# ZhangLearning/llm-message-queue

Measured on AMD Instinct MI355X. Metric: requests/sec + p99 enqueue->dispatch latency, 4-tier mix at 1/2/4/8 backends, higher is better.
Workload: dtype bf16

## Files before the change

### csrc/kernels/gemm_kernels.h

```cpp
#pragma once

#include <hip/hip_runtime.h>
#include <stdint.h>

#include <type_traits>

#include "fp8_decode.h"
#include "sample_noise.h"

namespace llmq {

typedef __attribute__((ext_vector_type(8))) short gm_bf16x8;
typedef __attribute__((ext_vector_type(4))) float gm_f32x4;
typedef __attribute__((ext_vector_type(4))) unsigned int gm_u32x4;

constexpr int GM_BM = 256, GM_BN = 256, GM_BK = 64, GM_THREADS = 512;
constexpr int GM_HALF_BYTES = 128 * GM_BK * 2;
constexpr int GM_BUF_BYTES = 4 * GM_HALF_BYTES;
constexpr int GM_LDS_BYTES = 2 * GM_BUF_BYTES;
constexpr int GM_GROUP_M = 8;

enum { GM_EPI_STORE = 0, GM_EPI_SWIGLU = 2, GM_EPI_ROPE = 3, GM_EPI_ARGMAX = 4, GM_EPI_RESID = 5,
       GM_EPI_RESID_LDS = 6, GM_EPI_RESID_PRE = 7, GM_EPI_RESID_RMS = 8, GM_EPI_SAMPLE = 9 };
constexpr int GM_LDS_SPARE = 32768;
template <int EPI>
constexpr int gm_lds_bytes() { return EPI == GM_EPI_RESID_PRE ? GM_LDS_BYTES + GM_LDS_SPARE : GM_LDS_BYTES; }

enum {
  GM_DIAG_NONE = 0,
  GM_DIAG_SKIP_A2 = 1,
  GM_DIAG_NO_LDS_READ = 2,
  GM_DIAG_NO_DMA = 3,
  GM_DIAG_CLOCK = 4,
  GM_DIAG_CLOCK_NO_DMA = 5,
  GM_DIAG_L2_PANELS = 6
};

struct GmSide {
  float* pv;
  int32_t* pi;
  union {
    float* rpart;
    const float* inv_temp;
  };
  union {
    int* rticket;
    const uint32_t* key;
  };
  float* rscale;
  float reps;
};

struct GmRope {
  const int32_t* pos;
  const int32_t* slot;
  const float* cos_t;
  const float* sin_t;
  uint16_t* q;
  uint16_t* kc;
  uint16_t* vc;
  int Hq, Hkv, max_ctx, n_slots;
};
enum { GM_A0 = 0, GM_A1 = 1, GM_B0 = 2, GM_B1 = 3 };

__device__ __forceinline__ uint16_t gm_f2bf(float f) {
  uint32_t u = __float_as_uint(f);
  u += 0x7fffu + ((u >> 16) & 1u);
  return (uint16_t)(u >> 16);
}

__device__ __forceinline__ void gm_load_row_scales(const float* __restrict__ rs, int row0, int fq,
                                                   gm_f32x4 (&sc)[2][4]) {
  if (rs) {
#pragma unroll
    for (int mh = 0; mh < 2; ++mh)
#pragma unroll
      for (int m = 0; m < 4; ++m)
        sc[mh][m] = *reinterpret_cast<const gm_f32x4*>(rs + row0 + mh * 64 + m * 16 + fq * 4);
  } else {
#pragma unroll
    for (int mh = 0; mh < 2; ++mh)
#pragma unroll
      for (int m = 0; m < 4; ++m) sc[mh][m] = gm_f32x4{1.f, 1.f, 1.f, 1.f};
  }
}

#define GM_CPOL_SC1 16

struct GmSplit {
  int full;
  float* ws;
  int* cnt;
};

typedef __attribute__((address_space(3))) void* gm_lds_ptr;
typedef gm_f32x4 gm_acc_t[2][4][2][2];

__device__ __forceinline__ void gm_stage(__amdgpu_buffer_rsrc_t rs, uint32_t v0, uint32_t v1, uint32_t soff,
                                         uint8_t* smem, uint32_t dst0, uint32_t dst1) {
  __builtin_amdgcn_raw_ptr_buffer_load_lds(rs, (gm_lds_ptr)(smem + dst0), 16, v0, soff, 0, 0);
  __builtin_amdgcn_raw_ptr_buffer_load_lds(rs, (gm_lds_ptr)(smem + dst1), 16, v1, soff, 0, 0);
}

#define GM_LGKM(N) asm volatile("s_waitcnt lgkmcnt(" #N ")" ::: "memory")
#define GM_VMCNT(N) asm volatile("s_waitcnt vmcnt(%0)" ::"n"(N) : "memory")
#define GM_FENCE() __builtin_amdgcn_sched_barrier(0)
#define GM_BARRIER()                  \
  do {                                \
    GM_FENCE();                       \
    __builtin_amdgcn_s_barrier();     \
    GM_FENCE();                       \
  } while (0)

typedef __attribute__((ext_vector_type(2))) unsigned int gf_u32x2;
template <int OFF>
__device__ __forceinline__ gf_u32x2 gf_lds_read_b64(uint32_t addr) {
  gf_u32x2 r;
  asm volatile("ds_read_b64 %0, %1 offset:%2" : "=v"(r) : "v"(addr), "n"(OFF) : "memory");
  return r;
}

template <int PER>
__device__ __forceinline__ int gm_xcd_run_start(int b, int count) {
  const int n = PER * count;
  const int xcd = b & 7, q8 = n >> 3, r8 = n & 7;
  return xcd < r8 ? xcd * (q8 + 1) : r8 * (q8 + 1) + (xcd - r8) * q8;
}

struct GmTile {
  int tm, tn;
  int pid;
// ... 54 lines not shown
    for (int spin = 0; spin < (1 << 24); ++spin) {
      if (__hip_atomic_load(cnt + 1, __ATOMIC_RELAXED, __HIP_MEMORY_SCOPE_AGENT)) break;
      __builtin_amdgcn_s_sleep(2);
    }
    GM_VMCNT(0);
    __hip_atomic_store(cnt, 0, __ATOMIC_RELAXED, __HIP_MEMORY_SCOPE_AGENT);
    __hip_atomic_store(cnt + 1, 0, __ATOMIC_RELAXED, __HIP_MEMORY_SCOPE_AGENT);
  }
  __syncthreads();
#pragma unroll
  for (int a = 0; a < 2; ++a)
#pragma unroll
    for (int b = 0; b < 4; ++b)
#pragma unroll
      for (int c = 0; c < 2; ++c)
#pragma unroll
        for (int d = 0; d < 2; ++d)
        {
          const int i = ((a * 4 + b) * 4 + c * 2 + d) * GM_THREADS + tid;
          acc[a][b][c][d] += __builtin_bit_cast(gm_f32x4, __builtin_amdgcn_raw_buffer_load_b128(
                                 srs, i * 16, 0, GM_CPOL_SC1));
        }
  return false;
}


template <int EPI, int DIAG, bool FP8 = false>
__device__ __forceinline__ void gemm_tile(
    uint8_t* __restrict__ smem, const uint16_t* __restrict__ A, const void* __restrict__ W,
    const float* __restrict__ cs, uint16_t* __restrict__ C, int M, int N, int K, int group_m,
    const float* __restrict__ rs, const GmRope& rp, const GmSplit& sp, const GmSide& am, const int bid) {
  static_assert(!FP8 || (DIAG == GM_DIAG_NONE &&
                         (EPI == GM_EPI_STORE || EPI == GM_EPI_SWIGLU || EPI == GM_EPI_RESID_LDS)),
                "the FP8 form: STORE, SWIGLU and RESID_LDS, no diagnostics");
  constexpr int kBHalf = 128 * GM_BK * (FP8 ? 1 : 2);
  constexpr int kBuf = 2 * GM_HALF_BYTES + 2 * kBHalf;
  static_assert(2 * kBuf <= GM_LDS_BYTES, "operand buffers inside the launch's LDS");
  constexpr bool kStamp = DIAG == GM_DIAG_CLOCK || DIAG == GM_DIAG_CLOCK_NO_DMA;
  const int tiles_m = (M + GM_BM - 1) / GM_BM;
  const int tiles_n = N / GM_BN;
  const int nwg = tiles_m * tiles_n;
  const int full = sp.ws ? sp.full : nwg;
  const GmTile tile = gm_tile_coords(bid, tiles_m, tiles_n, nwg, full, group_m);
  const int pid = tile.pid, khalf = tile.khalf, tm = tile.tm, tn = tile.tn;

  const int tid = threadIdx.x;
  const int lane = tid & 63;
  const int w = __builtin_amdgcn_readfirstlane(tid >> 6);
  uint64_t st_t0 = 0, st_r0 = 0;
  if constexpr (kStamp) {
    st_t0 = __builtin_amdgcn_s_memtime();
    st_r0 = __builtin_amdgcn_s_memrealtime();
  }
  const int wr = w >> 2, wc = w & 3;

  const int srow = w * 8 + (lane >> 3);
  const int schunk = (lane & 7) ^ ((srow >> 1) & 7);
  const int brow = w * 16 + (lane >> 2);
  const int bchunk = (lane & 3) ^ ((brow >> 2) & 3);
  const __amdgpu_buffer_rsrc_t rsa = __builtin_amdgcn_make_buffer_rsrc((void*)A, 0, M * K * 2, 0x00020000);
  const __amdgpu_buffer_rsrc_t rsw =
      __builtin_amdgcn_make_buffer_rsrc((void*)W, 0, N * K * (FP8 ? 1 : 2), 0x00020000);
  uint32_t va[2][2], vb[2][FP8 ? 1 : 2];
  const int ltm = DIAG == GM_DIAG_L2_PANELS ? 0 : tm, ltn = DIAG == GM_DIAG_L2_PANELS ? 0 : tn;
#pragma unroll
  for (int h = 0; h < 2; ++h) {
#pragma unroll
    for (int i = 0; i < 2; ++i) {
      int row = ltm * GM_BM + i * 128 + h * 64 + srow;
      row = row < M ? row : M - 1;
      va[h][i] = (uint32_t)row * (uint32_t)K * 2u + (uint32_t)schunk * 16u;
      if constexpr (!FP8) {
        const int col = ltn * GM_BN + (2 * i + (w >> 2)) * 64 + h * 32 + (w & 3) * 8 + (lane >> 3);
        vb[h][i] = (uint32_t)col * (uint32_t)K * 2u + (uint32_t)schunk * 16u;
      }
    }
    if constexpr (FP8) {
      const int col = ltn * GM_BN + (brow >> 5) * 64 + h * 32 + (brow & 31);
      vb[h][0] = (uint32_t)col * (uint32_t)K + (uint32_t)bchunk * 16u;
    }
  }
  const uint32_t dst_i0 = (uint32_t)(w * 8) * 128u;
  const uint32_t dst_i1 = (uint32_t)(64 + w * 8) * 128u;
  const uint32_t dst_b = (uint32_t)(w * 16) * 64u;

  const uint32_t sbase = (uint32_t)(uintptr_t)(__attribute__((address_space(3))) uint8_t*)smem;
  const int fr = lane & 15, fq = lane >> 4;
  uint32_t aoff[2][2], boff[2][2];
#pragma unroll
  for (int kk = 0; kk < 2; ++kk) {
    const int c = fq + 4 * kk;
    aoff[0][kk] = (uint32_t)(wr * 64 + fr) * 128u + (uint32_t)((c ^ ((fr >> 1) & 7)) * 16);
    if constexpr (FP8)
      boff[0][kk] = (uint32_t)(2 * GM_HALF_BYTES) + (uint32_t)(wc * 32 + fr) * 64u +
                    (uint32_t)(((c >> 1) ^ ((fr >> 2) & 3)) * 16 + (c & 1) * 8);
    else
      boff[0][kk] = (uint32_t)(wc * 32 + fr) * 128u + (uint32_t)((c ^ ((fr >> 1) & 7)) * 16) + 2 * GM_HALF_BYTES;
    aoff[1][kk] = aoff[0][kk] + kBuf;
    boff[1][kk] = boff[0][kk] + kBuf;
  }

  gm_acc_t acc;
#pragma unroll
  for (int a = 0; a < 2; ++a)
#pragma unroll
    for (int b = 0; b < 4; ++b)
// ... 38 lines not shown
      _Pragma("unroll") for (int kk = 0; kk < 2; ++kk) {                                       \
        DST[0][kk] = gf_lds_read_b64<(NH) * kBHalf>(sbase + boff[BUF][kk]);                    \
        DST[1][kk] = gf_lds_read_b64<(NH) * kBHalf + 1024>(sbase + boff[BUF][kk]);             \
      }                                                                                        \
    } else {                                                                                   \
      _Pragma("unroll") for (int n = 0; n < 2; ++n)                                            \
        _Pragma("unroll") for (int kk = 0; kk < 2; ++kk)                                       \
          DST[n][kk] = *reinterpret_cast<const gm_bf16x8*>(smem + boff[BUF][kk] + (NH) * kBHalf + n * 2048); \
    }                                                                                          \
  } while (0)
#define GM_READ_B(BUF, NH) GM_READ_B_INTO(BUF, NH, bfr[NH])
#define GM_READ_B0_INTO(BUF, DST) GM_READ_B_INTO(BUF, 0, DST)

#define GM_MFMA_WITH(MH, NH, BREG)                                                             \
  do {                                                                                         \
    _Pragma("unroll") for (int kk = 0; kk < 2; ++kk) {                                         \
      gm_bf16x8 _b[2];                                                                         \
      _Pragma("unroll") for (int n = 0; n < 2; ++n) {                                          \
        if constexpr (FP8) _b[n] = sk_fp8x8_bf16(BREG[n][kk].x, BREG[n][kk].y);                \
        else _b[n] = BREG[n][kk];                                                              \
      }                                                                                        \
      _Pragma("unroll") for (int m = 0; m < 4; ++m)                                            \
        _Pragma("unroll") for (int n = 0; n < 2; ++n)                                          \
          acc[MH][m][NH][n] = __builtin_amdgcn_mfma_f32_16x16x32_bf16(af[m][kk], _b[n],        \
                                                                      acc[MH][m][NH][n], 0, 0, 0); \
    }                                                                                          \
  } while (0)

#define GM_PHASE_END(MH, NH, BREG)   \
  do {                               \
    GM_BARRIER();                    \
    GM_LGKM(0);                      \
    if constexpr (FP8) GM_FENCE();   \
    GM_MFMA_WITH(MH, NH, BREG);      \
    GM_BARRIER();                    \
  } while (0)

  constexpr int kDmaA = 2, kDmaB = FP8 ? 1 : 2;
  constexpr int kFlyA = 2 * kDmaA + kDmaB, kFlyB = kDmaA + 2 * kDmaB;

  if (wr == 1) __builtin_amdgcn_s_setprio(1);
  if constexpr (EPI == GM_EPI_RESID_PRE) {
    const int col0p = tn * GM_BN + wc * 64, row0p = tm * GM_BM + wr * 128;
    const __amdgpu_buffer_rsrc_t rsp =
        __builtin_amdgcn_make_buffer_rsrc((void*)C, 0, (uint32_t)M * (uint32_t)N * 2u, 0x00020000);
#pragma unroll
    for (int i = 0; i < 4; ++i) {
      const int r = i * 8 + (lane >> 3), c = lane & 7;
      const uint32_t vo = ((uint32_t)(row0p + r) * (uint32_t)N + (uint32_t)(col0p + c * 8)) * 2u;
      __builtin_amdgcn_raw_ptr_buffer_load_lds(rsp, (gm_lds_ptr)(smem + GM_LDS_BYTES + w * 4096 + i * 1024), 16,
                                               vo, 0, 0, 0);
    }
  }
  GM_STAGE(0, GM_B0, 0);
  GM_STAGE(0, GM_A0, 0);
  GM_STAGE(0, GM_B1, 0);
  GM_STAGE(0, GM_A1, 0);
  GM_STAGE(1, GM_B0, 1);
  GM_STAGE(1, GM_A0, 1);
  GM_STAGE(1, GM_B1, 1);
  GM_VMCNT(kFlyB);
  GM_BARRIER();
  GM_READ_B0_INTO(0, bfr[0]);
  if constexpr (DIAG >= GM_DIAG_SKIP_A2 && DIAG <= GM_DIAG_NO_DMA) {
    GM_READ_A(0, 0);
    GM_READ_B(0, 1);
    GM_READ_B0_INTO(1, b0y);
  }
  if (wr == 1) GM_BARRIER();

  int t = 0;
  constexpr bool kRdA = DIAG != GM_DIAG_NO_LDS_READ;
  constexpr bool kRdA2 = DIAG != GM_DIAG_SKIP_A2 && DIAG != GM_DIAG_NO_LDS_READ;
  constexpr bool kRdB = DIAG != GM_DIAG_NO_LDS_READ;
  constexpr bool kDma = DIAG != GM_DIAG_NO_DMA && DIAG != GM_DIAG_CLOCK_NO_DMA;
#define GM_D_READ_A(ON, B, H) do { if constexpr (ON) GM_READ_A(B, H); } while (0)
#define GM_D_READ_B(B, H) do { if constexpr (kRdB) GM_READ_B(B, H); } while (0)
#define GM_D_READ_B0(B, D) do { if constexpr (kRdB) GM_READ_B0_INTO(B, D); } while (0)
#define GM_D_STAGE(B, H, K) do { if constexpr (kDma) GM_STAGE(B, H, K); } while (0)
  for (; t < nt - 2; t += 2) {
    {
      GM_D_READ_A(kRdA, 0, 0); GM_D_STAGE(1, GM_A1, t + 1); GM_VMCNT(kFlyA); GM_PHASE_END(0, 0, bfr[0]);
      GM_D_READ_B(0, 1); GM_D_STAGE(0, GM_B0, t + 2); GM_VMCNT(kFlyB); GM_PHASE_END(0, 1, bfr[1]);
      GM_D_READ_A(kRdA2, 0, 1); GM_D_STAGE(0, GM_A0, t + 2); GM_VMCNT(kFlyA); GM_PHASE_END(1, 1, bfr[1]);
      GM_D_READ_B0(1, b0y); GM_D_STAGE(0, GM_B1, t + 2); GM_VMCNT(kFlyB); GM_PHASE_END(1, 0, bfr[0]);
      GM_D_READ_A(kRdA, 1, 0); GM_D_STAGE(0, GM_A1, t + 2); GM_VMCNT(kFlyA); GM_PHASE_END(0, 0, b0y);
      GM_D_READ_B(1, 1); GM_D_STAGE(1, GM_B0, t + 3); GM_VMCNT(kFlyB); GM_PHASE_END(0, 1, bfr[1]);
      GM_D_READ_A(kRdA2, 1, 1); GM_D_STAGE(1, GM_A0, t + 3); GM_VMCNT(kFlyA); GM_PHASE_END(1, 1, bfr[1]);
      GM_D_READ_B0(0, bfr[0]); GM_D_STAGE(1, GM_B1, t + 3); GM_VMCNT(kFlyB); GM_PHASE_END(1, 0, b0y);
    }
  }
  {
      GM_READ_A(0, 0); GM_STAGE(1, GM_A1, t + 1); GM_VMCNT(kFlyA); GM_PHASE_END(0, 0, bfr[0]);
      GM_READ_B(0, 1); GM_VMCNT(kDmaA + kDmaB); GM_PHASE_END(0, 1, bfr[1]);
      GM_READ_A(0, 1); GM_VMCNT(kDmaA); GM_PHASE_END(1, 1, bfr[1]);
      GM_READ_B0_INTO(1, b0y); GM_VMCNT(0); GM_PHASE_END(1, 0, bfr[0]);
      GM_READ_A(1, 0); GM_PHASE_END(0, 0, b0y);
      GM_READ_B(1, 1); GM_PHASE_END(0, 1, bfr[1]);
      GM_READ_A(1, 1); GM_PHASE_END(1, 1, bfr[1]);
      GM_PHASE_END(1, 0, b0y);
  }
  __builtin_amdgcn_s_setprio(0);
  if (wr == 0) GM_BARRIER();
#undef GM_D_READ_A
#undef GM_D_READ_B
#undef GM_D_READ_B0
#undef GM_D_STAGE
#undef GM_PHASE_END
#undef GM_MFMA_WITH
#undef GM_READ_B0_INTO
#undef GM_READ_B
#undef GM_READ_B_INTO
#undef GM_READ_A
#undef GM_STAGE

  if (khalf >= 0 && gm_split_join(smem, acc, sp, pid - full)) return;

  if constexpr (FP8) {
    const float* csp = cs + tn * GM_BN + wc * 64 + fr;
#pragma unroll
    for (int nh = 0; nh < 2; ++nh)
#pragma unroll
      for (int n = 0; n < 2; ++n) {
        const float s = csp[nh * 32 + n * 16];
#pragma unroll
        for (int mh = 0; mh < 2; ++mh)
#pragma unroll
          for (int m = 0; m < 4; ++m) acc[mh][m][nh][n] *= s;
      }
  }

  const int row0 = tm * GM_BM + wr * 128;
  if constexpr (EPI == GM_EPI_ARGMAX || EPI == GM_EPI_SAMPLE) {
    if constexpr (EPI == GM_EPI_SAMPLE) {
      const uint32_t col = (uint32_t)(tn * GM_BN + wc * 64 + fr);
#pragma unroll
      for (int mh = 0; mh < 2; ++mh)
#pragma unroll
        for (int m = 0; m < 4; ++m) {
          const int r4 = row0 + mh * 64 + m * 16 + fq * 4;
          const gm_f32x4 it = *reinterpret_cast<const gm_f32x4*>(am.inv_temp + r4);
          const gm_u32x4 ka = *reinterpret_cast<const gm_u32x4*>(am.key + 2 * r4);
          const gm_u32x4 kb = *reinterpret_cast<const gm_u32x4*>(am.key + 2 * r4 + 4);
#pragma unroll
          for (int j = 0; j < 4; ++j) {
            const uint32_t k0 = j < 2 ? ka[2 * j] : kb[2 * j - 4];
            const uint32_t k1 = j < 2 ? ka[2 * j + 1] : kb[2 * j - 3];
            if (it[j] != 0.f) {
#pragma unroll
              for (int nh = 0; nh < 2; ++nh)
#pragma unroll
                for (int n = 0; n < 2; ++n)
                  acc[mh][m][nh][n][j] = acc[mh][m][nh][n][j] * it[j] + sn_gumbel(k0, k1, col + nh * 32 + n * 16);
            }
          }
        }
// ... 31 lines not shown
    if (tid < GM_BM) {
      const int grow = tm * GM_BM + tid;
      float v = lv[tid * 4];
      int c = lc[tid * 4];
#pragma unroll
      for (int k = 1; k < 4; ++k)
        if (lv[tid * 4 + k] > v) { v = lv[tid * 4 + k]; c = lc[tid * 4 + k]; }
      if (grow < M) {
        am.pv[(int64_t)grow * tiles_n + tn] = v;
        am.pi[(int64_t)grow * tiles_n + tn] = tn * GM_BN + c;
      }
    }
  } else if constexpr (EPI == GM_EPI_RESID) {
    float* o = reinterpret_cast<float*>(smem + w * (32 * 68 * 4));
    const int col0 = tn * GM_BN + wc * 64;
    uint2 cres[2][2][8];
#pragma unroll
    for (int mh = 0; mh < 2; ++mh)
#pragma unroll
      for (int mp = 0; mp < 2; ++mp)
#pragma unroll
        for (int it = 0; it < 8; ++it) {
          const int qd = it * 64 + lane;
          const int grow = row0 + mh * 64 + mp * 32 + (qd >> 4);
          cres[mh][mp][it] = grow < M ? *reinterpret_cast<const uint2*>(C + (int64_t)grow * N + col0 + (qd & 15) * 4)
                                      : make_uint2(0u, 0u);
        }
#pragma unroll
    for (int mh = 0; mh < 2; ++mh)
#pragma unroll
      for (int mp = 0; mp < 2; ++mp) {
#pragma unroll
        for (int mm = 0; mm < 2; ++mm)
#pragma unroll
          for (int nh = 0; nh < 2; ++nh)
#pragma unroll
            for (int n = 0; n < 2; ++n)
#pragma unroll
              for (int j = 0; j < 4; ++j)
                o[(mm * 16 + fq * 4 + j) * 68 + nh * 32 + n * 16 + fr] = acc[mh][mp * 2 + mm][nh][n][j];
        GM_LGKM(0);
        __builtin_amdgcn_wave_barrier();
#pragma unroll
        for (int it = 0; it < 8; ++it) {
          const int qd = it * 64 + lane;
          const int r = qd >> 4, c4 = qd & 15;
          const int grow = row0 + mh * 64 + mp * 32 + r;
          const gm_f32x4 v = *reinterpret_cast<const gm_f32x4*>(o + r * 68 + c4 * 4);
          if (grow < M) {
            uint2* cp = reinterpret_cast<uint2*>(C + (int64_t)grow * N + col0 + c4 * 4);
            const uint2 cr = cres[mh][mp][it];
            const float r0 = __uint_as_float(cr.x << 16) + v[0], r1 = __uint_as_float(cr.x & 0xffff0000u) + v[1];
            const float r2 = __uint_as_float(cr.y << 16) + v[2], r3 = __uint_as_float(cr.y & 0xffff0000u) + v[3];
            *cp = make_uint2((uint32_t)gm_f2bf(r0) | ((uint32_t)gm_f2bf(r1) << 16),
                             (uint32_t)gm_f2bf(r2) | ((uint32_t)gm_f2bf(r3) << 16));
          }
        }
        GM_LGKM(0);
        __builtin_amdgcn_wave_barrier();
      }
  } else if constexpr (EPI == GM_EPI_RESID_LDS || EPI == GM_EPI_RESID_PRE || EPI == GM_EPI_RESID_RMS) {
    constexpr int kPre = EPI == GM_EPI_RESID_PRE ? 4 : 0;
    uint8_t* cw = smem + w * 16384;
    uint8_t* cpre = smem + GM_LDS_BYTES + w * 4096;
    auto rowp = [&](int r) -> uint8_t* { return (kPre && r < 32) ? cpre + r * 128 : cw + r * 128; };
    const int col0 = tn * GM_BN + wc * 64;
    const __amdgpu_buffer_rsrc_t rsc =
        __builtin_amdgcn_make_buffer_rsrc((void*)C, 0, (uint32_t)M * (uint32_t)N * 2u, 0x00020000);
#pragma unroll
    for (int i = kPre; i < 16; ++i) {
      const int r = i * 8 + (lane >> 3), c = lane & 7;
      const uint32_t vo = ((uint32_t)(row0 + r) * (uint32_t)N + (uint32_t)(col0 + c * 8)) * 2u;
      __builtin_amdgcn_raw_ptr_buffer_load_lds(rsc, (gm_lds_ptr)(cw + i * 1024), 16, vo, 0, 0, 0);
    }
    GM_VMCNT(0);
    __builtin_amdgcn_wave_barrier();
#pragma unroll
    for (int mh = 0; mh < 2; ++mh)
#pragma unroll
      for (int m = 0; m < 4; ++m)
#pragma unroll
        for (int nh = 0; nh < 2; ++nh)
#pragma unroll
          for (int n = 0; n < 2; ++n)
#pragma unroll
            for (int j = 0; j < 4; ++j) {
              const int r = mh * 64 + m * 16 + fq * 4 + j;
              uint16_t* e = reinterpret_cast<uint16_t*>(rowp(r) + (nh * 32 + n * 16 + fr) * 2);
              *e = gm_f2bf(__uint_as_float((uint32_t)*e << 16) + acc[mh][m][nh][n][j]);
            }
    GM_LGKM(0);
    __builtin_amdgcn_wave_barrier();
    constexpr bool rms = EPI == GM_EPI_RESID_RMS;
    float ssq[16];
#pragma unroll
    for (int it = 0; it < 16; ++it) {
      const int qd = it * 64 + lane;
      const int r = qd >> 3, cb = qd & 7;
      const int grow = row0 + r;
      const gm_u32x4 v = *reinterpret_cast<const gm_u32x4*>(rowp(r) + cb * 16);
      if (grow < M) *reinterpret_cast<gm_u32x4*>(C + (int64_t)grow * N + col0 + cb * 8) = v;
      if constexpr (rms) {
        float q = 0.f;
#pragma unroll
        for (int e = 0; e < 4; ++e) {
          const float lo = __uint_as_float(v[e] << 16), hi = __uint_as_float(v[e] & 0xFFFF0000u);
          q += lo * lo + hi * hi;
        }
        ssq[it] = q;
      }
    }
    if constexpr (rms) {
#pragma unroll
      for (int it = 0; it < 16; ++it) {
        float q = ssq[it];
        q += __shfl_xor(q, 1, 64);
        q += __shfl_xor(q, 2, 64);
        q += __shfl_xor(q, 4, 64);
        ssq[it] = q;
      }
      GM_LGKM(0);
      __builtin_amdgcn_wave_barrier();
      float* wp = reinterpret_cast<float*>(cw);
      if ((lane & 7) == 0) {
#pragma unroll
        for (int it = 0; it < 16; ++it) wp[it * 8 + (lane >> 3)] = ssq[it];
      }
      __syncthreads();
      const int tiles_n_ = N / GM_BN;
      if (tid < 256) {
        const int hw = tid >> 7, rr = tid & 127;
        float sum = 0.f;
#pragma unroll
        for (int c = 0; c < 4; ++c) sum += reinterpret_cast<const float*>(smem + (hw * 4 + c) * 16384)[rr];
        const __amdgpu_buffer_rsrc_t prs = __builtin_amdgcn_make_buffer_rsrc(
            am.rpart + (size_t)(tm * tiles_n_ + tn) * 256, 0, 256 * 4, 0x00020000);
        __builtin_amdgcn_raw_buffer_store_b32(__float_as_uint(sum), prs, tid * 4, 0, GM_CPOL_SC1);
      }
      GM_VMCNT(0);
      __syncthreads();
      if (tid == 0)
        *reinterpret_cast<int*>(smem) = __hip_atomic_fetch_add(am.rticket + tm, 1, __ATOMIC_RELAXED,
                                                               __HIP_MEMORY_SCOPE_AGENT);
      __syncthreads();
      const int done = *reinterpret_cast<volatile int*>(smem);
      if (done == tiles_n_ - 1 && tid < 256) {
        float sum = 0.f;
        for (int t2 = 0; t2 < tiles_n_; ++t2) {
          const __amdgpu_buffer_rsrc_t prs = __builtin_amdgcn_make_buffer_rsrc(
              am.rpart + (size_t)(tm * tiles_n_ + t2) * 256, 0, 256 * 4, 0x00020000);
          sum += __uint_as_float(__builtin_amdgcn_raw_buffer_load_b32(prs, tid * 4, 0, GM_CPOL_SC1));
        }
        am.rscale[tm * 256 + tid] = rsqrtf(sum / (float)N + am.reps);
        if (tid == 0) __hip_atomic_store(am.rticket + tm, 0, __ATOMIC_RELAXED, __HIP_MEMORY_SCOPE_AGENT);
      }
    }
  } else if constexpr (EPI == GM_EPI_SWIGLU) {
    uint16_t* o = reinterpret_cast<uint16_t*>(smem + w * 8192);
    gm_f32x4 sc[2][4];
    gm_load_row_scales(rs, row0, fq, sc);
#pragma unroll
    for (int mh = 0; mh < 2; ++mh)
#pragma unroll
      for (int m = 0; m < 4; ++m)
#pragma unroll
        for (int n = 0; n < 2; ++n)
#pragma unroll
          for (int j = 0; j < 4; ++j) {
            const float g = acc[mh][m][0][n][j] * sc[mh][m][j];
            const float u = acc[mh][m][1][n][j] * sc[mh][m][j];
            const float s = g / (1.0f + __expf(-g));
            o[(mh * 64 + m * 16 + fq * 4 + j) * 32 + n * 16 + fr] = gm_f2bf(s * u);
          }
    GM_LGKM(0);
    __builtin_amdgcn_wave_barrier();
    const int F = N >> 1;
    const int col0 = tn * (GM_BN / 2) + wc * 32;
#pragma unroll
    for (int it = 0; it < 8; ++it) {
      const int qd = it * 64 + lane;
      const int r = qd >> 2, cb = qd & 3;
      const int grow = row0 + r;
      const gm_u32x4 v = *reinterpret_cast<const gm_u32x4*>(smem + w * 8192 + r * 64 + cb * 16);
      if (grow < M) *reinterpret_cast<gm_u32x4*>(C + (int64_t)grow * F + col0 + cb * 8) = v;
    }
  } else {
    uint16_t* o = reinterpret_cast<uint16_t*>(smem + w * 16384);
    gm_f32x4 sc[2][4];
    gm_load_row_scales(rs, row0, fq, sc);
#pragma unroll
    for (int mh = 0; mh < 2; ++mh)
#pragma unroll
      for (int m = 0; m < 4; ++m)
#pragma unroll
        for (int nh = 0; nh < 2; ++nh)
#pragma unroll
          for (int n = 0; n < 2; ++n)
#pragma unroll
            for (int j = 0; j < 4; ++j)
              o[(mh * 64 + m * 16 + fq * 4 + j) * 64 + nh * 32 + n * 16 + fr] =
                  gm_f2bf(acc[mh][m][nh][n][j] * sc[mh][m][j]);
    if constexpr (EPI == GM_EPI_STORE) {
      GM_LGKM(0);
      __builtin_amdgcn_wave_barrier();
      const int col0 = tn * GM_BN + wc * 64;
#pragma unroll
      for (int it = 0; it < 16; ++it) {
        const int qd = it * 64 + lane;
        const int r = qd >> 3, cb = qd & 7;
        const int grow = row0 + r;
        const gm_u32x4 v = *reinterpret_cast<const gm_u32x4*>(smem + w * 16384 + r * 128 + cb * 16);
        if (grow < M) *reinterpret_cast<gm_u32x4*>(C + (int64_t)grow * N + col0 + cb * 8) = v;
      }
    } else {
      __syncthreads();
      auto at = [&](int r, int c) -> const uint8_t* {
        return smem + ((r >> 7) * 4 + (c >> 6)) * 16384 + (r & 127) * 128 + (c & 63) * 2;
      };
      const int nq = rp.Hq / 2, nk = rp.Hkv / 2;
      if (tn < nq + nk) {
        const int hh = (tid >> 3) & 1, j = tid & 7, r0 = tid >> 4;
        int pk[8], sk[8];
#pragma unroll
        for (int k = 0; k < 8; ++k) {
          const int grow = min(tm * GM_BM + r0 + 32 * k, M - 1);
          pk[k] = rp.pos[grow];
          sk[k] = rp.slot[grow];
        }
        float4 c0[8], c1[8], s0[8], s1[8];
#pragma unroll
        for (int k = 0; k < 8; ++k) {
          const int64_t o = (int64_t)min(max(pk[k], 0), rp.max_ctx - 1) * 64 + 8 * j;
          c0[k] = *reinterpret_cast<const float4*>(rp.cos_t + o);
          c1[k] = *reinterpret_cast<const float4*>(rp.cos_t + o + 4);
          s0[k] = *reinterpret_cast<const float4*>(rp.sin_t + o);
          s1[k] = *reinterpret_cast<const float4*>(rp.sin_t + o + 4);
        }
#pragma unroll
        for (int k = 0; k < 8; ++k) {
          const int r = r0 + 32 * k;
          const int grow = tm * GM_BM + r;
          const int p = pk[k], sl = sk[k];
          if (grow >= M || (unsigned)sl >= (unsigned)rp.n_slots || (unsigned)p >= (unsigned)rp.max_ctx) continue;
          const gm_u32x4 lo = *reinterpret_cast<const gm_u32x4*>(at(r, hh * 128 + 8 * j));
          const gm_u32x4 hi = *reinterpret_cast<const gm_u32x4*>(at(r, hh * 128 + 64 + 8 * j));
          const float cc[8] = {c0[k].x, c0[k].y, c0[k].z, c0[k].w, c1[k].x, c1[k].y, c1[k].z, c1[k].w};
          const float ss[8] = {s0[k].x, s0[k].y, s0[k].z, s0[k].w, s1[k].x, s1[k].y, s1[k].z, s1[k].w};
          gm_u32x4 olo, ohi;
#pragma unroll
          for (int e = 0; e < 4; ++e) {
            const float a0 = __uint_as_float(lo[e] << 16), a1 = __uint_as_float(lo[e] & 0xffff0000u);
            const float b0 = __uint_as_float(hi[e] << 16), b1 = __uint_as_float(hi[e] & 0xffff0000u);
            const float c_0 = cc[2 * e], c_1 = cc[2 * e + 1], s_0 = ss[2 * e], s_1 = ss[2 * e + 1];
            olo[e] = (uint32_t)gm_f2bf(a0 * c_0 - b0 * s_0) | ((uint32_t)gm_f2bf(a1 * c_1 - b1 * s_1) << 16);
            ohi[e] = (uint32_t)gm_f2bf(b0 * c_0 + a0 * s_0) | ((uint32_t)gm_f2bf(b1 * c_1 + a1 * s_1) << 16);
          }
          uint16_t* dst;
          if (tn < nq) {
            dst = rp.q + (int64_t)grow * rp.Hq * 128 + (2 * tn + hh) * 128;
          } else {
            const int kvh = 2 * (tn - nq) + hh;
            dst = rp.kc + (((int64_t)sl * rp.Hkv + kvh) * rp.max_ctx + p) * 128;
          }
          *reinterpret_cast<gm_u32x4*>(dst + 8 * j) = olo;
          *reinterpret_cast<gm_u32x4*>(dst + 64 + 8 * j) = ohi;
        }
      } else {
        const int hh = (tid >> 4) & 1, cb = tid & 15, r0 = tid >> 5;
        int pk[16], sk[16];
#pragma unroll
        for (int k = 0; k < 16; ++k) {
          const int grow = min(tm * GM_BM + r0 + 16 * k, M - 1);
          pk[k] = rp.pos[grow];
          sk[k] = rp.slot[grow];
        }
        const int kvh = 2 * (tn - nq - nk) + hh;
#pragma unroll
        for (int k = 0; k < 16; ++k) {
          const int r = r0 + 16 * k;
          const int grow = tm * GM_BM + r;
          const int p = pk[k], sl = sk[k];
          if (grow >= M || (unsigned)sl >= (unsigned)rp.n_slots || (unsigned)p >= (unsigned)rp.max_ctx) continue;
          uint16_t* dst = rp.vc + (((int64_t)sl * rp.Hkv + kvh) * rp.max_ctx + p) * 128;
          *reinterpret_cast<gm_u32x4*>(dst + 8 * cb) = *reinterpret_cast<const gm_u32x4*>(at(r, hh * 128 + 8 * cb));
        }
      }
    }
  }
  if constexpr (kStamp) {
    const uint64_t st_t1 = __builtin_amdgcn_s_memtime(), st_r1 = __builtin_amdgcn_s_memrealtime();
    if (tid == 0 && am.pv != nullptr) {
      uint64_t* dbg = reinterpret_cast<uint64_t*>(am.pv) + (size_t)bid * 4;
      dbg[0] = st_t0;
      dbg[1] = st_t1;
      dbg[2] = st_r0;
      dbg[3] = st_r1;
    }
  }
}

template <int EPI, int DIAG = GM_DIAG_NONE>
__global__ __launch_bounds__(GM_THREADS) void gemm_bf16_kernel(
    const uint16_t* __restrict__ A, const uint16_t* __restrict__ W, uint16_t* __restrict__ C,
    int M, int N, int K, int group_m, const float* __restrict__ rs, const GmRope rp, const GmSplit sp,
    const GmSide am) {
  extern __shared__ __align__(16) uint8_t smem[];
  gemm_tile<EPI, DIAG>(smem, A, W, nullptr, C, M, N, K, group_m, rs, rp, sp, am, (int)blockIdx.x);
}

template <int EPI>
__global__ __launch_bounds__(GM_THREADS) void gemm_fp8w_kernel(
    const uint16_t* __restrict__ A, const uint8_t* __restrict__ Wq, const float* __restrict__ cs,
    uint16_t* __restrict__ C, int M, int N, int K, int group_m, const float* __restrict__ rs, const GmSplit sp) {
  extern __shared__ __align__(16) uint8_t smem[];
  gemm_tile<EPI, GM_DIAG_NONE, true>(smem, A, Wq, cs, C, M, N, K, group_m, rs, GmRope{}, sp, GmSide{},
                                     (int)blockIdx.x);
}

__global__ __launch_bounds__(256) void gemm_argmax_reduce_kernel(const float* __restrict__ pv,
                                                                 const int32_t* __restrict__ pi, int M, int tiles,
                                                                 int32_t* __restrict__ out) {
  const int row = blockIdx.x * 4 + (threadIdx.x >> 6);
  const int lane = threadIdx.x & 63;
  if (row >= M) return;
  float v = -__builtin_inff();
  int c = 0x7fffffff;
  for (int t = lane; t < tiles; t += 64) {
    const float x = pv[(int64_t)row * tiles + t];
    if (x > v) { v = x; c = pi[(int64_t)row * tiles + t]; }
  }
#pragma unroll
  for (int off = 1; off < 64; off <<= 1) {
    const float ov = __shfl_xor(v, off, 64);
    const int oc = __shfl_xor(c, off, 64);
    if (ov > v || (ov == v && oc < c)) { v = ov; c = oc; }
  }
  if (lane == 0) out[row] = c == 0x7fffffff ? 0 : c;
}

__global__ __launch_bounds__(256) void sample_bits_kernel(const uint32_t* __restrict__ keys, uint32_t n0, int count,
                                                          uint32_t* __restrict__ out) {
  const int i = blockIdx.x * 256 + threadIdx.x;
  const int k = blockIdx.y;
  if (i < count) out[(int64_t)k * count + i] = sn_bits(keys[2 * k], keys[2 * k + 1], n0 + (uint32_t)i);
}

#undef GM_LGKM
#undef GM_VMCNT
#undef GM_BARRIER
#undef GM_FENCE

// ... 2 lines not shown
```

### csrc/kernels/skinny_kernels.h

```cpp
#pragma once
#include <hip/hip_runtime.h>
#include <stdint.h>

#include <type_traits>

#include "fp8_decode.h"

namespace llmq {

typedef __attribute__((ext_vector_type(4))) float sk_f32x4;

constexpr int SK_NB = 128;
constexpr int SK_KS = 128;
constexpr int SK_LDA = SK_KS + 8;

enum { SK_EPI_STORE = 0, SK_EPI_RESID = 1, SK_EPI_SWIGLU = 2 };

constexpr int SK_MAX_M = 1024;

template <bool FP8>
struct SkW {
  using elem = std::conditional_t<FP8, uint8_t, uint16_t>;
  static constexpr int ST = FP8 ? 5 : 3;
  static constexpr int NV = FP8 ? 2 : 4;
// ... 81 lines not shown
    if (more) load_a(step + 1);
    const int abuf = step & 1;
#pragma unroll
    for (int s4 = 0; s4 < 4; ++s4) {
      sk_bf16x8 b0, b1;
      if constexpr (FP8) {
        b0 = sk_fp8x8_bf16(wb[CUR][0][s4 >> 1][(s4 & 1) * 2], wb[CUR][0][s4 >> 1][(s4 & 1) * 2 + 1]);
        b1 = sk_fp8x8_bf16(wb[CUR][1][s4 >> 1][(s4 & 1) * 2], wb[CUR][1][s4 >> 1][(s4 & 1) * 2 + 1]);
      } else {
        b0 = __builtin_bit_cast(sk_bf16x8, wb[CUR][0][s4]);
        b1 = __builtin_bit_cast(sk_bf16x8, wb[CUR][1][s4]);
      }
#pragma unroll
      for (int m = 0; m < MT; ++m) {
        const sk_bf16x8 a = *reinterpret_cast<const sk_bf16x8*>(&As[abuf][m * 16 + fr][(fq * 4 + s4) * 8]);
        acc[m][0] = __builtin_amdgcn_mfma_f32_16x16x32_bf16(a, b0, acc[m][0], 0, 0, 0);
        acc[m][1] = __builtin_amdgcn_mfma_f32_16x16x32_bf16(a, b1, acc[m][1], 0, 0, 0);
      }
    }
    if (more) store_a(abuf ^ 1);
    __syncthreads();
  };

  load_a(0);
  load_w(std::integral_constant<int, 0>{}, 0);
  if (nsteps > 1) load_w(std::integral_constant<int, 1>{}, 1);
  if constexpr (ST > 3) {
    if (nsteps > 2) load_w(std::integral_constant<int, 2>{}, 2);
    if (nsteps > 3) load_w(std::integral_constant<int, 3>{}, 3);
  }
  store_a(0);
  __syncthreads();
  for (int step = 0; step < nsteps; step += ST) {
    run_step(std::integral_constant<int, 0>{}, step);
    if (step + 1 < nsteps) run_step(std::integral_constant<int, 1>{}, step + 1);
    if (step + 2 < nsteps) run_step(std::integral_constant<int, 2>{}, step + 2);
    if constexpr (ST > 3) {
      if (step + 3 < nsteps) run_step(std::integral_constant<int, 3>{}, step + 3);
      if (step + 4 < nsteps) run_step(std::integral_constant<int, 4>{}, step + 4);
    }
  }
  float* out = ws + (size_t)blockIdx.y * M * N;
#pragma unroll
  for (int m = 0; m < MT; ++m)
#pragma unroll
    for (int j = 0; j < 2; ++j)
#pragma unroll
      for (int e = 0; e < 4; ++e) {
        const int row = m * 16 + fq * 4 + e;
        if (row < Ml) out[(size_t)(m0 + row) * N + n0 + j * 16 + fr] = acc[m][j][e];
      }
}

__device__ __forceinline__ uint16_t sk_f2bf(float f) {
  uint32_t u = __float_as_uint(f);
  u += 0x7fffu + ((u >> 16) & 1u);
  return (uint16_t)(u >> 16);
}

template <int EPI, bool COLS>
__device__ __forceinline__ void sk_finalize(const float* __restrict__ ws, int S, int M, int N,
                                            const float* __restrict__ rs, const float* __restrict__ cs,
                                            uint16_t* __restrict__ C) {
  const int Nout = EPI == SK_EPI_SWIGLU ? N / 2 : N;
  const int per_row = Nout / 4;
  const int gid = blockIdx.x * 256 + threadIdx.x;
  if (gid >= M * per_row) return;
  const int row = gid / per_row, c4 = (gid % per_row) * 4;
  const float scale = rs ? rs[row] : 1.f;
  if constexpr (EPI == SK_EPI_SWIGLU) {
    const int t = c4 / 128, wc = (c4 % 128) / 32, c = c4 % 32;
    const int gcol = t * 256 + wc * 64 + c;
    sk_f32x4 g = sk_f32x4{0.f, 0.f, 0.f, 0.f}, u = g;
    for (int s = 0; s < S; ++s) {
      const float* p = ws + ((size_t)s * M + row) * N;
      g += *reinterpret_cast<const sk_f32x4*>(p + gcol);
      u += *reinterpret_cast<const sk_f32x4*>(p + gcol + 32);
    }
    if constexpr (COLS) {
      g *= *reinterpret_cast<const sk_f32x4*>(cs + gcol);
      u *= *reinterpret_cast<const sk_f32x4*>(cs + gcol + 32);
    }
    uint16_t o[4];
#pragma unroll
    for (int e = 0; e < 4; ++e) {
      const float ge = g[e] * scale, ue = u[e] * scale;
      o[e] = sk_f2bf(ge / (1.f + __expf(-ge)) * ue);
    }
    *reinterpret_cast<uint2*>(C + (size_t)row * Nout + c4) =
        make_uint2((uint32_t)o[0] | ((uint32_t)o[1] << 16), (uint32_t)o[2] | ((uint32_t)o[3] << 16));
  } else {
    sk_f32x4 v = sk_f32x4{0.f, 0.f, 0.f, 0.f};
    for (int s = 0; s < S; ++s) v += *reinterpret_cast<const sk_f32x4*>(ws + ((size_t)s * M + row) * N + c4);
    if constexpr (COLS) v *= *reinterpret_cast<const sk_f32x4*>(cs + c4);
    uint2* cp = reinterpret_cast<uint2*>(C + (size_t)row * N + c4);
    float r[4] = {v[0] * scale, v[1] * scale, v[2] * scale, v[3] * scale};
    if constexpr (EPI == SK_EPI_RESID) {
      const uint2 cr = *cp;
      r[0] += __uint_as_float(cr.x << 16);
      r[1] += __uint_as_float(cr.x & 0xffff0000u);
      r[2] += __uint_as_float(cr.y << 16);
      r[3] += __uint_as_float(cr.y & 0xffff0000u);
    }
    *cp = make_uint2((uint32_t)sk_f2bf(r[0]) | ((uint32_t)sk_f2bf(r[1]) << 16),
                     (uint32_t)sk_f2bf(r[2]) | ((uint32_t)sk_f2bf(r[3]) << 16));
  }
}

template <int EPI>
__global__ void __launch_bounds__(256)
skinny_finalize_kernel(const float* __restrict__ ws, int S, int M, int N, const float* __restrict__ rs,
                       uint16_t* __restrict__ C) {
  sk_finalize<EPI, false>(ws, S, M, N, rs, nullptr, C);
}

template <int EPI>
__global__ void __launch_bounds__(256)
skinny_finalize_cs_kernel(const float* __restrict__ ws, int S, int M, int N, const float* __restrict__ rs,
                          const float* __restrict__ cs, uint16_t* __restrict__ C) {
  sk_finalize<EPI, true>(ws, S, M, N, rs, cs, C);
}

__global__ void __launch_bounds__(256) fp8_decode_kernel(const uint32_t* __restrict__ in, int n,
                                                         uint16_t* __restrict__ out) {
  const int i = blockIdx.x * 256 + threadIdx.x;
  if (i >= n) return;
  const uint32_t w = in[i >> 2];
  const uint32_t p = (i & 2) ? sk_fp8x2_bf16<true>(w) : sk_fp8x2_bf16<false>(w);
  out[i] = (uint16_t)((i & 1) ? p >> 16 : p);
}

__device__ __forceinline__ uint32_t sk_e4m3_rne(float x) {
  const uint32_t b = __float_as_uint(x), sign = (b >> 24) & 0x80u;
  uint32_t u = b & 0x7fffffffu;
  if (u >= 0x3c800000u) {
    u += 0x7ffffu + ((u >> 20) & 1u);
    return sign | ((u >> 20) - (120u << 3));
  }
  const float f = __uint_as_float(u) + 16384.f;
  return sign | (__float_as_uint(f) - 0x46800000u);
}

__global__ void __launch_bounds__(256)
quant_rows_e4m3_kernel(const uint16_t* __restrict__ W, int K, uint8_t* __restrict__ codes, float* __restrict__ scale) {
  __shared__ uint32_t red[4];
  const uint16_t* wr = W + (size_t)blockIdx.x * K;
  uint8_t* cr = codes + (size_t)blockIdx.x * K;
  const int nv = K / 8;
  uint32_t amax = 0;
  for (int v = threadIdx.x; v < nv; v += 256) {
    const sk_u32x4 x = *reinterpret_cast<const sk_u32x4*>(wr + v * 8);
#pragma unroll
    for (int i = 0; i < 4; ++i) amax = max(amax, max(x[i] & 0x7fffu, (x[i] >> 16) & 0x7fffu));
  }
#pragma unroll
  for (int o = 32; o > 0; o >>= 1) amax = max(amax, (uint32_t)__shfl_xor((int)amax, o));
  if ((threadIdx.x & 63) == 0) red[threadIdx.x >> 6] = amax;
  __syncthreads();
// ... 26 lines not shown
```

Baseline: 5348.

## Prefetch epilogue row scales and RoPE pos/slot into LDS; use packed bf16 conversion

Row scales, and for the RoPE epilogue also the position and slot indices, are now loaded into a new LDS region by async buffer-to-LDS DMA at kernel start. This takes global loads off the epilogue's critical path. Float-to-bf16 conversion now converts two values at a time through a vector __bf16 convert, which can map to packed hardware conversion on gfx950, in both the GEMM and skinny kernels. The change also adds a phase-timestamp diagnostic mode and enlarges LDS use for the affected epilogues, which may affect occupancy. The conversion rounding for NaN cases may differ from the old manual round-to-nearest-even.

```diff
diff --git a/csrc/kernels/gemm_kernels.h b/csrc/kernels/gemm_kernels.h
--- a/csrc/kernels/gemm_kernels.h
+++ b/csrc/kernels/gemm_kernels.h
@@ -23,8 +23,14 @@
 enum { GM_EPI_STORE = 0, GM_EPI_SWIGLU = 2, GM_EPI_ROPE = 3, GM_EPI_ARGMAX = 4, GM_EPI_RESID = 5,
        GM_EPI_RESID_LDS = 6, GM_EPI_RESID_PRE = 7, GM_EPI_RESID_RMS = 8, GM_EPI_SAMPLE = 9 };
 constexpr int GM_LDS_SPARE = 32768;
+constexpr int GM_ROWIN_SCALE = 0, GM_ROWIN_POS = 1024, GM_ROWIN_SLOT = 2048, GM_ROWIN_BYTES = 3072;
 template <int EPI>
-constexpr int gm_lds_bytes() { return EPI == GM_EPI_RESID_PRE ? GM_LDS_BYTES + GM_LDS_SPARE : GM_LDS_BYTES; }
+constexpr bool gm_row_inputs() { return EPI == GM_EPI_STORE || EPI == GM_EPI_SWIGLU || EPI == GM_EPI_ROPE; }
+template <int EPI>
+constexpr int gm_lds_bytes() {
+  return EPI == GM_EPI_RESID_PRE ? GM_LDS_BYTES + GM_LDS_SPARE
+                                 : gm_row_inputs<EPI>() ? GM_LDS_BYTES + GM_ROWIN_BYTES : GM_LDS_BYTES;
+}
 
 enum {
   GM_DIAG_NONE = 0,
@@ -33,7 +39,8 @@
   GM_DIAG_NO_DMA = 3,
   GM_DIAG_CLOCK = 4,
   GM_DIAG_CLOCK_NO_DMA = 5,
-  GM_DIAG_L2_PANELS = 6
+  GM_DIAG_L2_PANELS = 6,
+  GM_DIAG_PHASES = 7
 };
 
 struct GmSide {
@@ -63,20 +70,20 @@
 };
 enum { GM_A0 = 0, GM_A1 = 1, GM_B0 = 2, GM_B1 = 3 };
 
-__device__ __forceinline__ uint16_t gm_f2bf(float f) {
-  uint32_t u = __float_as_uint(f);
-  u += 0x7fffu + ((u >> 16) & 1u);
-  return (uint16_t)(u >> 16);
-}
-
-__device__ __forceinline__ void gm_load_row_scales(const float* __restrict__ rs, int row0, int fq,
-                                                   gm_f32x4 (&sc)[2][4]) {
-  if (rs) {
+typedef __attribute__((ext_vector_type(2))) float gm_f32x2;
+typedef __attribute__((ext_vector_type(2))) __bf16 gm_bf16x2;
+__device__ __forceinline__ uint32_t gm_f2bf(float lo, float hi) {
+  return __builtin_bit_cast(uint32_t, __builtin_convertvector(gm_f32x2{lo, hi}, gm_bf16x2));
+}
+
+__device__ __forceinline__ void gm_lds_row_scales(const uint8_t* __restrict__ smem, bool have, int wr, int fq,
+                                                  gm_f32x4 (&sc)[2][4]) {
+  if (have) {
+    const float* ls = reinterpret_cast<const float*>(smem + GM_LDS_BYTES + GM_ROWIN_SCALE) + wr * 128 + fq * 4;
 #pragma unroll
     for (int mh = 0; mh < 2; ++mh)
 #pragma unroll
-      for (int m = 0; m < 4; ++m)
-        sc[mh][m] = *reinterpret_cast<const gm_f32x4*>(rs + row0 + mh * 64 + m * 16 + fq * 4);
+      for (int m = 0; m < 4; ++m) sc[mh][m] = *reinterpret_cast<const gm_f32x4*>(ls + mh * 64 + m * 16);
   } else {
 #pragma unroll
     for (int mh = 0; mh < 2; ++mh)
@@ -237,6 +244,18 @@
     st_t0 = __builtin_amdgcn_s_memtime();
     st_r0 = __builtin_amdgcn_s_memrealtime();
   }
+  constexpr bool kPhase = DIAG == GM_DIAG_PHASES;
+  uint64_t ph_t[5] = {0, 0, 0, 0, 0}, ph_r0 = 0;
+#define GM_PHASE_STAMP(I)                           \
+  do {                                              \
+    if constexpr (kPhase) {                         \
+      GM_FENCE();                                   \
+      ph_t[I] = __builtin_amdgcn_s_memtime();       \
+      GM_FENCE();                                   \
+    }                                               \
+  } while (0)
+  if constexpr (kPhase) ph_r0 = __builtin_amdgcn_s_memrealtime();
+  GM_PHASE_STAMP(0);
   const int wr = w >> 2, wc = w & 3;
 
   const int srow = w * 8 + (lane >> 3);
@@ -381,6 +400,21 @@
                                                vo, 0, 0, 0);
     }
   }
+  if constexpr (gm_row_inputs<EPI>()) {
+    if (w == 0 && rs != nullptr) {
+      const __amdgpu_buffer_rsrc_t rsr =
+          __builtin_amdgcn_make_buffer_rsrc((void*)rs, 0, tiles_m * GM_BM * 4, 0x00020000);
+      __builtin_amdgcn_raw_ptr_buffer_load_lds(rsr, (gm_lds_ptr)(smem + GM_LDS_BYTES + GM_ROWIN_SCALE), 16,
+                                               (uint32_t)(tm * GM_BM * 4 + lane * 16), 0, 0, 0);
+    }
+    if constexpr (EPI == GM_EPI_ROPE) {
+      static_assert(GM_ROWIN_SLOT == GM_ROWIN_POS + GM_BM * 4, "pos then slot, 64 rows a wave");
+      const __amdgpu_buffer_rsrc_t rsi =
+          __builtin_amdgcn_make_buffer_rsrc((void*)(w < 4 ? rp.pos : rp.slot), 0, M * 4, 0x00020000);
+      __builtin_amdgcn_raw_ptr_buffer_load_lds(rsi, (gm_lds_ptr)(smem + GM_LDS_BYTES + GM_ROWIN_POS + w * 256), 4,
+                                               (uint32_t)((tm * GM_BM + (w & 3) * 64 + lane) * 4), 0, 0, 0);
+    }
+  }
   GM_STAGE(0, GM_B0, 0);
   GM_STAGE(0, GM_A0, 0);
   GM_STAGE(0, GM_B1, 0);
@@ -390,6 +424,7 @@
   GM_STAGE(1, GM_B1, 1);
   GM_VMCNT(kFlyB);
   GM_BARRIER();
+  GM_PHASE_STAMP(1);
   GM_READ_B0_INTO(0, bfr[0]);
   if constexpr (DIAG >= GM_DIAG_SKIP_A2 && DIAG <= GM_DIAG_NO_DMA) {
     GM_READ_A(0, 0);
@@ -431,6 +466,7 @@
   }
   __builtin_amdgcn_s_setprio(0);
   if (wr == 0) GM_BARRIER();
+  GM_PHASE_STAMP(2);
 #undef GM_D_READ_A
 #undef GM_D_READ_B
 #undef GM_D_READ_B0
@@ -568,8 +604,7 @@
             const uint2 cr = cres[mh][mp][it];
             const float r0 = __uint_as_float(cr.x << 16) + v[0], r1 = __uint_as_float(cr.x & 0xffff0000u) + v[1];
             const float r2 = __uint_as_float(cr.y << 16) + v[2], r3 = __uint_as_float(cr.y & 0xffff0000u) + v[3];
-            *cp = make_uint2((uint32_t)gm_f2bf(r0) | ((uint32_t)gm_f2bf(r1) << 16),
-                             (uint32_t)gm_f2bf(r2) | ((uint32_t)gm_f2bf(r3) << 16));
+            *cp = make_uint2(gm_f2bf(r0, r1), gm_f2bf(r2, r3));
           }
         }
         GM_LGKM(0);
@@ -600,13 +635,18 @@
 #pragma unroll
           for (int n = 0; n < 2; ++n)
 #pragma unroll
-            for (int j = 0; j < 4; ++j) {
+            for (int j = 0; j < 4; j += 2) {
               const int r = mh * 64 + m * 16 + fq * 4 + j;
-              uint16_t* e = reinterpret_cast<uint16_t*>(rowp(r) + (nh * 32 + n * 16 + fr) * 2);
-              *e = gm_f2bf(__uint_as_float((uint32_t)*e << 16) + acc[mh][m][nh][n][j]);
+              uint16_t* e0 = reinterpret_cast<uint16_t*>(rowp(r) + (nh * 32 + n * 16 + fr) * 2);
+              uint16_t* e1 = reinterpret_cast<uint16_t*>(rowp(r + 1) + (nh * 32 + n * 16 + fr) * 2);
+              const uint32_t p = gm_f2bf(__uint_as_float((uint32_t)*e0 << 16) + acc[mh][m][nh][n][j],
+                                         __uint_as_float((uint32_t)*e1 << 16) + acc[mh][m][nh][n][j + 1]);
+              *e0 = (uint16_t)p;
+              *e1 = (uint16_t)(p >> 16);
             }
     GM_LGKM(0);
     __builtin_amdgcn_wave_barrier();
+    GM_PHASE_STAMP(3);
     constexpr bool rms = EPI == GM_EPI_RESID_RMS;
     float ssq[16];
 #pragma unroll
@@ -674,7 +714,7 @@
   } else if constexpr (EPI == GM_EPI_SWIGLU) {
     uint16_t* o = reinterpret_cast<uint16_t*>(smem + w * 8192);
     gm_f32x4 sc[2][4];
-    gm_load_row_scales(rs, row0, fq, sc);
+    gm_lds_row_scales(smem, rs != nullptr, wr, fq, sc);
 #pragma unroll
     for (int mh = 0; mh < 2; ++mh)
 #pragma unroll
@@ -682,14 +722,23 @@
 #pragma unroll
         for (int n = 0; n < 2; ++n)
 #pragma unroll
-          for (int j = 0; j < 4; ++j) {
-            const float g = acc[mh][m][0][n][j] * sc[mh][m][j];
-            const float u = acc[mh][m][1][n][j] * sc[mh][m][j];
-            const float s = g / (1.0f + __expf(-g));
-            o[(mh * 64 + m * 16 + fq * 4 + j) * 32 + n * 16 + fr] = gm_f2bf(s * u);
+          for (int j = 0; j < 4; j += 2) {
+            float h[2];
+#pragma unroll
+            for (int jj = 0; jj < 2; ++jj) {
+              const float g = acc[mh][m][0][n][j + jj] * sc[mh][m][j + jj];
+              const float u = acc[mh][m][1][n][j + jj] * sc[mh][m][j + jj];
+              const float s = g / (1.0f + __expf(-g));
+              h[jj] = s * u;
+            }
+            const uint32_t p = gm_f2bf(h[0], h[1]);
+            uint16_t* e = o + (mh * 64 + m * 16 + fq * 4 + j) * 32 + n * 16 + fr;
+            e[0] = (uint16_t)p;
+            e[32] = (uint16_t)(p >> 16);
           }
     GM_LGKM(0);
     __builtin_amdgcn_wave_barrier();
+    GM_PHASE_STAMP(3);
     const int F = N >> 1;
     const int col0 = tn * (GM_BN / 2) + wc * 32;
 #pragma unroll
@@ -703,7 +752,7 @@
   } else {
     uint16_t* o = reinterpret_cast<uint16_t*>(smem + w * 16384);
     gm_f32x4 sc[2][4];
-    gm_load_row_scales(rs, row0, fq, sc);
+    gm_lds_row_scales(smem, rs != nullptr, wr, fq, sc);
 #pragma unroll
     for (int mh = 0; mh < 2; ++mh)
 #pragma unroll
@@ -713,12 +762,17 @@
 #pragma unroll
           for (int n = 0; n < 2; ++n)
 #pragma unroll
-            for (int j = 0; j < 4; ++j)
-              o[(mh * 64 + m * 16 + fq * 4 + j) * 64 + nh * 32 + n * 16 + fr] =
-                  gm_f2bf(acc[mh][m][nh][n][j] * sc[mh][m][j]);
+            for (int j = 0; j < 4; j += 2) {
+              const uint32_t p = gm_f2bf(acc[mh][m][nh][n][j] * sc[mh][m][j],
+                                         acc[mh][m][nh][n][j + 1] * sc[mh][m][j + 1]);
+              uint16_t* e = o + (mh * 64 + m * 16 + fq * 4 + j) * 64 + nh * 32 + n * 16 + fr;
+              e[0] = (uint16_t)p;
+              e[64] = (uint16_t)(p >> 16);
+            }
     if constexpr (EPI == GM_EPI_STORE) {
       GM_LGKM(0);
       __builtin_amdgcn_wave_barrier();
+      GM_PHASE_STAMP(3);
       const int col0 = tn * GM_BN + wc * 64;
 #pragma unroll
       for (int it = 0; it < 16; ++it) {
@@ -730,18 +784,20 @@
       }
     } else {
       __syncthreads();
+      GM_PHASE_STAMP(3);
       auto at = [&](int r, int c) -> const uint8_t* {
         return smem + ((r >> 7) * 4 + (c >> 6)) * 16384 + (r & 127) * 128 + (c & 63) * 2;
       };
       const int nq = rp.Hq / 2, nk = rp.Hkv / 2;
+      const int* lpos = reinterpret_cast<const int*>(smem + GM_LDS_BYTES + GM_ROWIN_POS);
+      const int* lslot = reinterpret_cast<const int*>(smem + GM_LDS_BYTES + GM_ROWIN_SLOT);
       if (tn < nq + nk) {
         const int hh = (tid >> 3) & 1, j = tid & 7, r0 = tid >> 4;
         int pk[8], sk[8];
 #pragma unroll
         for (int k = 0; k < 8; ++k) {
-          const int grow = min(tm * GM_BM + r0 + 32 * k, M - 1);
-          pk[k] = rp.pos[grow];
-          sk[k] = rp.slot[grow];
+          pk[k] = lpos[r0 + 32 * k];
+          sk[k] = lslot[r0 + 32 * k];
         }
         float4 c0[8], c1[8], s0[8], s1[8];
 #pragma unroll
@@ -768,8 +824,8 @@
             const float a0 = __uint_as_float(lo[e] << 16), a1 = __uint_as_float(lo[e] & 0xffff0000u);
             const float b0 = __uint_as_float(hi[e] << 16), b1 = __uint_as_float(hi[e] & 0xffff0000u);
             const float c_0 = cc[2 * e], c_1 = cc[2 * e + 1], s_0 = ss[2 * e], s_1 = ss[2 * e + 1];
-            olo[e] = (uint32_t)gm_f2bf(a0 * c_0 - b0 * s_0) | ((uint32_t)gm_f2bf(a1 * c_1 - b1 * s_1) << 16);
-            ohi[e] = (uint32_t)gm_f2bf(b0 * c_0 + a0 * s_0) | ((uint32_t)gm_f2bf(b1 * c_1 + a1 * s_1) << 16);
+            olo[e] = gm_f2bf(a0 * c_0 - b0 * s_0, a1 * c_1 - b1 * s_1);
+            ohi[e] = gm_f2bf(b0 * c_0 + a0 * s_0, b1 * c_1 + a1 * s_1);
           }
           uint16_t* dst;
           if (tn < nq) {
@@ -786,9 +842,8 @@
         int pk[16], sk[16];
 #pragma unroll
         for (int k = 0; k < 16; ++k) {
-          const int grow = min(tm * GM_BM + r0 + 16 * k, M - 1);
-          pk[k] = rp.pos[grow];
-          sk[k] = rp.slot[grow];
+          pk[k] = lpos[r0 + 16 * k];
+          sk[k] = lslot[r0 + 16 * k];
         }
         const int kvh = 2 * (tn - nq - nk) + hh;
 #pragma unroll
@@ -813,6 +868,18 @@
       dbg[3] = st_r1;
     }
   }
+  if constexpr (kPhase) {
+    GM_PHASE_STAMP(4);
+    const uint64_t ph_r4 = __builtin_amdgcn_s_memrealtime();
+    if (tid == 0 && am.pv != nullptr) {
+      uint64_t* dbg = reinterpret_cast<uint64_t*>(am.pv) + (size_t)bid * 8;
+#pragma unroll
+      for (int i = 0; i < 5; ++i) dbg[i] = ph_t[i];
+      dbg[5] = ph_r0;
+      dbg[6] = ph_r4;
+    }
+  }
+#undef GM_PHASE_STAMP
 }
 
 template <int EPI, int DIAG = GM_DIAG_NONE>
diff --git a/csrc/kernels/skinny_kernels.h b/csrc/kernels/skinny_kernels.h
--- a/csrc/kernels/skinny_kernels.h
+++ b/csrc/kernels/skinny_kernels.h
@@ -157,10 +157,10 @@
       }
 }
 
-__device__ __forceinline__ uint16_t sk_f2bf(float f) {
-  uint32_t u = __float_as_uint(f);
-  u += 0x7fffu + ((u >> 16) & 1u);
-  return (uint16_t)(u >> 16);
+typedef __attribute__((ext_vector_type(2))) float sk_f32x2;
+typedef __attribute__((ext_vector_type(2))) __bf16 sk_bf16x2;
+__device__ __forceinline__ uint32_t sk_f2bf(float lo, float hi) {
+  return __builtin_bit_cast(uint32_t, __builtin_convertvector(sk_f32x2{lo, hi}, sk_bf16x2));
 }
 
 template <int EPI, bool COLS>
@@ -186,14 +186,13 @@
       g *= *reinterpret_cast<const sk_f32x4*>(cs + gcol);
       u *= *reinterpret_cast<const sk_f32x4*>(cs + gcol + 32);
     }
-    uint16_t o[4];
+    float o[4];
 #pragma unroll
     for (int e = 0; e < 4; ++e) {
       const float ge = g[e] * scale, ue = u[e] * scale;
-      o[e] = sk_f2bf(ge / (1.f + __expf(-ge)) * ue);
-    }
-    *reinterpret_cast<uint2*>(C + (size_t)row * Nout + c4) =
-        make_uint2((uint32_t)o[0] | ((uint32_t)o[1] << 16), (uint32_t)o[2] | ((uint32_t)o[3] << 16));
+      o[e] = ge / (1.f + __expf(-ge)) * ue;
+    }
+    *reinterpret_cast<uint2*>(C + (size_t)row * Nout + c4) = make_uint2(sk_f2bf(o[0], o[1]), sk_f2bf(o[2], o[3]));
   } else {
     sk_f32x4 v = sk_f32x4{0.f, 0.f, 0.f, 0.f};
     for (int s = 0; s < S; ++s) v += *reinterpret_cast<const sk_f32x4*>(ws + ((size_t)s * M + row) * N + c4);
@@ -207,8 +206,7 @@
       r[2] += __uint_as_float(cr.y << 16);
       r[3] += __uint_as_float(cr.y & 0xffff0000u);
     }
-    *cp = make_uint2((uint32_t)sk_f2bf(r[0]) | ((uint32_t)sk_f2bf(r[1]) << 16),
-                     (uint32_t)sk_f2bf(r[2]) | ((uint32_t)sk_f2bf(r[3]) << 16));
+    *cp = make_uint2(sk_f2bf(r[0], r[1]), sk_f2bf(r[2], r[3]));
   }
 }
 
```

New measurement: 5356 (median of 2 runs). About the same (+0.1%).
